# osmocom/osmo-trx

Hardware: AMD Instinct MI355X
Metric: Mbursts/s detect+demod (156.25 sym, 4 SPS) (higher is better)
Workload: dtype f32

## Files before the change

osmo_trx_amd/csrc/trx_device.h:

```cpp
#pragma once
#include <hip/hip_runtime.h>
#include <stdint.h>
#include <stdlib.h>
#include <atomic>

#include "trx_tables.h"
#include "../../include/trxhip.h"

#define WAVE 64
#define TRX_PAD 20
#define TRX_DEC_LEN 208
#define TRX_CORR_MAX 128
#define TRX_DEC_NARROW 160
#define TRX_CORR_NARROW 80
#define TRX_CZ_PAD 12
#define TRX_CZ_LEN (TRX_CZ_PAD + TRX_CORR_MAX + TRX_CZ_PAD)
#define TRX_SINCV_LDS (TRX_SINCV_LEN + 32)
#define TRX_CLIP_THRESH 30000.0f
#define TRX_WPB 12

#define LSEQ_TSC(s)   ((s) * 16)
#define LSEQ_RACH(i)  (128 + (i) * 40)
#define LSEQ_EDGE(s)  (248 + (s) * 16)
#define LSEQ_DUMMY    376
// ... 395 lines not shown
		p.y += v.y * w[u];
	}
	return p;
}

__device__ __forceinline__ int sinc_base_lo(int f) { return trx_sincv_swz(f); }
__device__ __forceinline__ int sinc_base_hi(int f) { return (f == 0) ? 512 : trx_sincv_swz(512 - f); }

__device__ __forceinline__ c32 interp_point(const c32 *cz, int ix512, const float *sincv)
{
	const int fl = ix512 >> 9;
	const int f = ix512 & 511;
	return interp_taps(cz + (fl - 7), sincv + sinc_base_lo(f), sincv + sinc_base_hi(f));
}

struct PeakConst {
	int flA;
	int loA, hiA;
	int offB;
	int ratio_off;
};
__device__ __forceinline__ int node_offset(int n, int inc0);
__device__ __forceinline__ PeakConst peak_const(int lane)
{
	PeakConst pc;
	const int offA = node_offset(lane >> 1, 256) + ((lane & 1) ? 1024 : 0);
	pc.flA = offA >> 9;
	pc.loA = sinc_base_lo(offA & 511);
	pc.hiA = sinc_base_hi(offA & 511);
	pc.offB = (lane < 32) ? node_offset(lane >> 1, 8) + ((lane & 1) ? 1024 : 0) : (2 * (lane & 15) - 15) + 512;
// ... 31 lines not shown
	int off = 0;
#pragma unroll
	for (int Lw = 0; Lw < LEVELS; Lw++) {
		const unsigned bit = 2u * node;
		const unsigned l = (unsigned)(lt >> bit) & 1u;
		stop |= (unsigned)(eq >> bit) & 1u;
		const int step = inc0 >> Lw;
		const int delta = l ? step : -step;
		off += stop ? 0 : delta;
		node = 2u * node + 1u + l;
	}
	tie = stop != 0u;
	return off;
}

__device__ __forceinline__ void peak_detect_spec(const c32 *cz, int max_idx, const float *sincv, const PeakConst &pc,
						  int lane, int *toa512_out, c32 *val_out, const float4 *wa4 = nullptr)
{
	int E = (max_idx - 1) * 512;
	bool tie = false;

	{
		const c32 *const ca = cz + ((max_idx - 1) + pc.flA - 7);
		const float nv = wa4 ? norm2(interp_taps_w(ca, wa4[lane], wa4[64 + lane], wa4[128 + lane], wa4[192 + lane]))
				     : norm2(interp_taps(ca, sincv + pc.loA, sincv + pc.hiA));
		E += walk_tree<5>(nv, 256, tie);
	}
	int final_ix;
	c32 val;
	if (!tie) {
		const c32 pv = interp_point(cz, E + pc.offB, sincv);
		const float nv = norm2(pv);
		const int offB = walk_tree<4>(nv, 8, tie);
		E += offB;
		final_ix = E + 512;
		const int src = 32 + ((offB + 15) >> 1);
		val.x = lane_val(pv.x, src);
		val.y = lane_val(pv.y, src);
	}
	if (tie) {
		final_ix = E + 512;
		val = interp_point(cz, final_ix, sincv);
	}
	*toa512_out = final_ix;
	*val_out = val;
}

#define TRX_FAST_W      2.6f
#define TRX_FAST_KAPPA  6e-6f
static __device__ unsigned long long g_trx_fast_stats[4];

__device__ __forceinline__ trx_v2f pk_fma_w(trx_v2f x, float w, trx_v2f acc)
{
	return __builtin_elementwise_fma(x, (trx_v2f){ w, w }, acc);
}

__device__ __forceinline__ c32 interp_taps_fma(const c32 *c, const float *sa, const float *sb)
// ... 506 lines not shown
```

osmo_trx_amd/csrc/trx_kernel_nb.hip:

```cpp
#include "trx_k4_common.h"
#include "trx_nb_asm.inc"

#define NB_D_LEN    160
#define NB_CZ_LEN   (TRX_CZ_PAD + TRX_CORR_NARROW + TRX_CZ_PAD)
#define NB_SLICE    (K4_XS + NB_D_LEN + NB_CZ_LEN)
#define NB_COMP_ROWS (TRX_DELAY_FILTS + 1)
#define NB_TABLES_FLOATS (TRX_SINCV_LDS + 16 * WAVE + NB_COMP_ROWS * 36 + 16 + 8 * 8 + 5 * WAVE + 5 * WAVE + 2 * 8 * 16)
#define NB_TABLES_BYTES (NB_TABLES_FLOATS * 4)
#define NB_WPB 16
#define NB_POOL_RING 64
#define NB_POOL_UNSET (-1)
#define NB_POOL_END (-2)
#define NB_NO_BURST 0xffffffffu
#define NB_LDS_TAIL (16 + 4 * NB_POOL_RING)
#define NB_LDS_BYTES (NB_TABLES_BYTES + NB_WPB * NB_SLICE * 8 + NB_LDS_TAIL)
#define NB_MAX_TOA 32



typedef float v3f __attribute__((ext_vector_type(3)));
typedef int v4i __attribute__((ext_vector_type(4)));
typedef __attribute__((address_space(3))) v2f lds_v2f;

template <typename T>
__device__ __forceinline__ unsigned lds_addr(const T *p)
{
	return (unsigned)(uintptr_t)(const __attribute__((address_space(3))) T *)p;
}

__device__ __forceinline__ int nb_lane_id()
{
	int lane;
	asm volatile("v_mbcnt_lo_u32_b32 %0, -1, 0\n\tv_mbcnt_hi_u32_b32 %0, -1, %0" : "=v"(lane));
	return lane;
}

// ... 19 lines not shown
	float *const wa4f = sincv + TRX_SINCV_LDS;
	const float4 *const wa4 = reinterpret_cast<const float4 *>(wa4f);
	float *const comp = wa4f + 16 * WAVE;
	float *const gdec = comp + NB_COMP_ROWS * 36;
	float *const lhdr = gdec + 16;
	int *const pkcl = reinterpret_cast<int *>(lhdr + 8 * 8);
	int *const lcn = pkcl + 5 * WAVE;
	c32 *const lseq = reinterpret_cast<c32 *>(lcn + 5 * WAVE);
	c32 *const wbase = reinterpret_cast<c32 *>(smem + NB_TABLES_BYTES) + (size_t)wave * NB_SLICE;
	int *const wg_next = reinterpret_cast<int *>(reinterpret_cast<c32 *>(smem + NB_TABLES_BYTES) + (size_t)NB_WPB * NB_SLICE);
	int *const pool_g = wg_next + 4;
	c32 *const P = wbase;
	c32 *const D = wbase + K4_XS;
	c32 *const cz = D + NB_D_LEN + TRX_CZ_PAD;

	for (int i = threadIdx.x; i < TRX_SINCV_LDS; i += blockDim.x)
		sincv[i] = (i < TRX_SINCV_LEN) ? tab->sincv[i] : 0.0f;
	for (int i = threadIdx.x; i < 16 * WAVE; i += blockDim.x) {
		const int l = i & (WAVE - 1), u = i >> 6;
		const PeakConst pcl = peak_const(l);
		const int q = (u < 8) ? pcl.loA + 512 * (7 - u) : pcl.hiA + 512 * (u - 8);
		wa4f[((u >> 2) * WAVE + l) * 4 + (u & 3)] = (q < TRX_SINCV_LEN) ? tab->sincv[q] : 0.0f;
	}
	for (int i = threadIdx.x; i < NB_COMP_ROWS * 36; i += blockDim.x) {
		const int f = i / 36, j = i % 36;
		comp[i] = (j >= TRX_FUSED_SH) ? tab->comp_filt[f][j - TRX_FUSED_SH] : 0.0f;
	}
	if (threadIdx.x < 16)
		gdec[threadIdx.x] = tab->dec_taps[threadIdx.x];
	if (threadIdx.x < 128)
		lseq[threadIdx.x] = make_float2(tab->seq[TRX_SEQ_TSC0 + (threadIdx.x >> 4)].taps[threadIdx.x & 15].re,
						tab->seq[TRX_SEQ_TSC0 + (threadIdx.x >> 4)].taps[threadIdx.x & 15].im);
	if (threadIdx.x < 64)
		lhdr[threadIdx.x] = reinterpret_cast<const float *>(&tab->seq[TRX_SEQ_TSC0 + (threadIdx.x >> 3)].gain)[threadIdx.x & 7];
	if (threadIdx.x < WAVE) {
		const PeakConst pc0 = peak_const(threadIdx.x);
		pkcl[0 * WAVE + threadIdx.x] = pc0.flA;
		pkcl[1 * WAVE + threadIdx.x] = pc0.loA;
		pkcl[2 * WAVE + threadIdx.x] = pc0.hiA;
		pkcl[3 * WAVE + threadIdx.x] = pc0.offB;
		pkcl[4 * WAVE + threadIdx.x] = pc0.ratio_off;
		lcn[0 * WAVE + threadIdx.x] = pc0.ratio_off * 8;
		lcn[1 * WAVE + threadIdx.x] = (pc0.flA - 8) * 8;
		lcn[2 * WAVE + threadIdx.x] = pc0.offB;
		const int l = threadIdx.x, e = (l - 52) / 3, t = (l - 52) % 3;
		const bool sp = l >= 52;
		lcn[3 * WAVE + l] = 8 * (sp ? (t == 0 ? e : t == 1 ? e + 3 : e - 3) : 4 + 3 * (l < 49 ? l : 49));
		lcn[4 * WAVE + l] = sp ? (e + (t == 2 ? 4 : 0)) * K4_NTP * 4 : -1;
	}
	for (int i = lane0; i < NB_SLICE; i += WAVE)
		wbase[i] = make_float2(0.0f, 0.0f);
	if (threadIdx.x == 0) {
		wg_next[0] = NB_WPB;
		wg_next[1] = 0;
	}
	if (threadIdx.x < NB_POOL_RING)
		pool_g[threadIdx.x] = NB_POOL_UNSET;
	__syncthreads();

	const float thr2 = thresh * thresh;
	float gkv = lane0 == 5 ? gk5 : lane0 == 6 ? gk6 : lane0 == 7 ? gk7 : gk8;
	asm volatile("" : "+v"(gkv));
// ... 338 lines not shown
			{
				int clip;
				asm("s_cmp_lg_u64 %1, 0\n\ts_cselect_b32 %0, 1, 0" : "=s"(clip) : "s"(__ballot(amax > TRX_CLIP_THRESH)) : "scc");

				const int len = 16 + (int)max_toa;
				__builtin_assume(len >= 16 && len <= 16 + NB_MAX_TOA);
				float v;
				const int lag0 = (len <= NB_ASM_CORR_MAX_LEN) ? NB_ASM_CORR_LANE0 : 0;
				asm volatile(NB_ASM_DECCORR
					     : [nrm] "=&v"(v)
					     : [aw] "v"(a_w), [zero] "v"(0), [len] "s"(len), [tsc] "s"(tsc)
					     : NB_ASM_CLOBBERS);
				{
					DIAG_MARK(3);
					int m_bits, es_bits, bidx;
					int kr, ka, kb, kic, ktp;
					asm volatile(NB_ASM_AMAX("ds_read_b32 %[kr], %[l4] offset:%c[lc]", "ds_read_b32 %[ka], %[l4] offset:%c[lc]+256",
								 "ds_read_b32 %[kb], %[l4] offset:%c[lc]+512", "ds_read_b32 %[kic], %[l4] offset:%c[lc]+768",
								 "ds_read_b32 %[ktp], %[l4] offset:%c[lc]+1024", "s_nop 0", "s_nop 0", "s_nop 0")
						     "s_sub_u32 %[bidx], %[bidx], %[lag0]\n\t"
						     "s_waitcnt lgkmcnt(0)"
						     : [m] "=&s"(m_bits), [es] "=&s"(es_bits), [bidx] "=&s"(bidx), [kr] "=&v"(kr), [ka] "=&v"(ka), [kb] "=&v"(kb),
						       [kic] "=&v"(kic), [ktp] "=&v"(ktp)
						     : [nrm] "v"(v), [ep] "v"(epart), [l4] "v"(a_l4), [lag0] "s"(lag0),
						       [lc] "n"((TRX_SINCV_LDS + 16 * WAVE + NB_COMP_ROWS * 36 + 16 + 64 + 5 * WAVE) * 4)
						     : NB_ASM_CLOBBERS);
					DIAG_MARK(4);
					int st, e512;
					float km;
					asm volatile(NB_ASM_DETA
						     : [st] "=&" NB_ASM_ST(st), [e] "=&s"(e512), [km] "=&v"(km)
						     : [bidx] "s"(bidx), [len] "s"(len), [czb] "s"(lds_addr(cz)), [kr] "v"(kr), [ka] "v"(ka), [l16] "v"(a_l16),
						       [gkv] "v"(gkv), [c0] "v"(gc0)
						     : NB_ASM_CLOBBERS_ST);
					DIAG_MARK(5);
					int toa512 = 0, xr_bits = 0, xi_bits = 0;
					if (__builtin_expect(st == 1, 1)) {
						asm volatile(NB_ASM_DETB
							     : [st] "=&" NB_ASM_ST(st), [toa] "=&s"(toa512), [xr] "=&s"(xr_bits), [xi] "=&s"(xi_bits)
							     : [e] "s"(e512), [kb] "v"(kb), [czb] "s"(lds_addr(cz)), [km] "v"(km)
							     : NB_ASM_CLOBBERS_ST);
						DIAG_MARK(6);
					}
					if (__builtin_expect(st != 1, 0)) {
						int stc = st;
						asm volatile("" : "+s"(stc));
						if (stc == 3) {
							const int lane = nb_lane_id();
							if (lane == 0)
								atomicAdd(&g_trx_fast_stats[0], 1ull);
							PeakConst pkc;
							pkc.flA = pkcl[0 * WAVE + lane]; pkc.loA = pkcl[1 * WAVE + lane]; pkc.hiA = pkcl[2 * WAVE + lane];
							pkc.offB = pkcl[3 * WAVE + lane]; pkc.ratio_off = pkcl[4 * WAVE + lane];
							c32 xcorr;
							peak_detect_spec(cz, bidx, sincv, pkc, lane, &toa512, &xcorr, wa4);
							toa512 = uni(toa512);
							xr_bits = uni(__float_as_int(xcorr.x));
							xi_bits = uni(__float_as_int(xcorr.y));
							st = 1;
						} else if (stc == 2) {
							if (nb_lane_id() == 0) atomicAdd(&g_trx_fast_stats[2], 1ull);
							mark_left(b);
							keep = 0;
						} else {
							const float energy = __int_as_float(es_bits) * 0.0125f;
							const float rssi = rssi_db(full_scale, energy);
							const uint32_t flags = ((uint32_t)clip << 8) | (1u << 16);
							int word = clip ? -TRXHIP_SIGERR_CLIP : 0;
							word = put_lane<1>(word, 0.0f);
							word = put_lane<2>(word, 0.0f);
// ... 5 lines not shown
							recw = word;
							o = (v3f){ 0.0f, 0.0f, 0.0f };
							pend_rm = 0xff;
						}
					}
					if (__builtin_expect(st == 1, 1)) {
						int ok, s_bits;
						float d0, d1, d2;
						const int t5 = (t5pk << (28 - 4 * tsc)) >> 28;
						asm volatile("s_setprio 0");
						asm volatile(NB_ASM_TAIL
							     : [ok] "=&s"(ok), [ssum] "=&s"(s_bits), [d0] "=&v"(d0), [d1] "=&v"(d1), [d2] "=&v"(d2)
							     : [toa] "s"(toa512), [xr] "s"(xr_bits), [xi] "s"(xi_bits), [t5] "s"(t5), [hdrb] "s"(lds_addr(lhdr) + 32u * (unsigned)tsc),
							       [e8lo] "s"((unsigned)e8_addr), [e8hi] "s"((unsigned)(e8_addr >> 32)), [l16] "v"(a_l16),
							       [aw] "v"(a_w), [pb] "s"(lds_addr(P)), [cb] "s"(lds_addr(comp) + 4u * (K4_U0 + TRX_FUSED_SH)), [db] "s"(lds_addr(D)),
							       [kic] "v"(kic), [ktp] "v"(ktp)
							     : NB_ASM_CLOBBERS);
						DIAG_MARK(10);
						asm volatile("s_setprio 2");
						o.x = __builtin_amdgcn_fmed3f(fmaf(0.5f, d0, 0.5f), 0.0f, 1.0f);
						o.y = __builtin_amdgcn_fmed3f(fmaf(0.5f, d1, 0.5f), 0.0f, 1.0f);
						o.z = __builtin_amdgcn_fmed3f(fmaf(0.5f, d2, 0.5f), 0.0f, 1.0f);
						queue_record(xr_bits, xi_bits, es_bits, toa512 - t5 - 10 * 512, s_bits,
							     (int)((uint32_t)tsc | ((uint32_t)clip << 8) | (37u << 24)), b);
						if (__builtin_expect(!ok, 0)) {
							const int lane = nb_lane_id();
							if (lane == 0) atomicAdd(&g_trx_fast_stats[3], 1ull);
							const float *const h = lhdr + 8 * tsc;
							const float xr = __int_as_float(xr_bits), xi = __int_as_float(xi_bits);
							const float a0 = xr * h[2], a1 = xr * h[3], a2 = xi * h[3], a3 = xi * h[2];
							const c32 ampv = make_float2(unif(a0 - a2), unif(a1 + a3));
							if (!demod_general(t5 + 10 * 512 - toa512, ampv, lane)) {
								q_n--;
								mark_left(b);
								keep = 0;
							}
						}
// ... 28 lines not shown
```

osmo_trx_amd/csrc/trx_nb_asm.inc:

```
#define NB_ASM_GDEC_OFF 29968
#define NB_ASM_LSEQ_OFF 32848
#define NB_ASM_DEC_MAX_NACT 60
#define NB_ASM_CORR_LANE0 19
#define NB_ASM_CORR_MAX_LEN 45
#define NB_ASM_AW_PD 512
#define NB_ASM_AW_D 5760
#define NB_ASM_AW_CZ 7136
#define NB_ASM_ST "{s98}"
#define NB_ASM_CLOBBERS "v64", "v65", "v66", "v67", "v68", "v69", "v70", "v71", "v72", "v73", "v74", "v75", "v76", "v77", "v78", "v79", "v80", "v81", "v82", "v83", "v84", "v85", "v86", "v87", "v88", "v89", "v90", "v91", "v92", "v93", "v94", "v95", "v96", "v97", "v98", "v99", "v100", "v101", "v102", "v103", "v104", "v105", "v106", "v107", "v108", "v109", "v110", "v111", "v112", "v113", "v114", "v115", "v116", "v117", "v118", "v119", "v120", "v121", "v122", "v123", "v124", "v125", "v126", "v127", "s87", "s88", "s89", "s90", "s91", "s92", "s93", "s94", "s95", "s96", "s97", "s98", "s99", "vcc", "scc", "memory"
#define NB_ASM_CLOBBERS_ST "v64", "v65", "v66", "v67", "v68", "v69", "v70", "v71", "v72", "v73", "v74", "v75", "v76", "v77", "v78", "v79", "v80", "v81", "v82", "v83", "v84", "v85", "v86", "v87", "v88", "v89", "v90", "v91", "v92", "v93", "v94", "v95", "v96", "v97", "v98", "v99", "v100", "v101", "v102", "v103", "v104", "v105", "v106", "v107", "v108", "v109", "v110", "v111", "v112", "v113", "v114", "v115", "v116", "v117", "v118", "v119", "v120", "v121", "v122", "v123", "v124", "v125", "v126", "v127", "s87", "s88", "s89", "s90", "s91", "s92", "s93", "s94", "s95", "s96", "s97", "s99", "vcc", "scc", "memory"
#define NB_ASM_DECCORR \
	"s_add_u32 s92, %[len], 15\n\t" \
	"s_cmp_gt_u32 %[len], 45\n\t" \
	"s_cbranch_scc1 .Lnbc_dc_wide\n\t" \
	"s_sub_u32 s88, 60, s92\n\t" \
	"s_lshr_b64 exec, -1, s88\n\t" \
	"ds_read_b128 v[120:123], %[zero] offset:29968\n\t" \
	"ds_read_b128 v[124:127], %[zero] offset:29984\n\t" \
	"ds_read_b64 v[98:99], %[aw] offset:1952\n\t" \
	"ds_read_b64 v[100:101], %[aw] offset:3392\n\t" \
	"ds_read_b64 v[102:103], %[aw] offset:4832\n\t" \
	"ds_read_b64 v[96:97], %[aw] offset:512\n\t" \
	"s_waitcnt lgkmcnt(3)\n\t" \
	"v_pk_mul_f32 v[64:65], v[98:99], v[120:121] op_sel:[0,0] op_sel_hi:[1,0]\n\t" \
// ... 1278 lines not shown
	".Lnb_da_end:\n\t"
#define NB_ASM_DETB \
	"v_mov_b64_e32 v[64:65], 0\n\t" \
	"v_mov_b64_e32 v[66:67], 0\n\t" \
	"v_add_u32_e32 v68, %[e], %[kb]\n\t" \
	"s_add_u32 s88, %[czb], -56\n\t" \
	"s_mov_b32 exec_lo, 0x3fffffff\n\t" \
	"s_mov_b32 exec_hi, 0xffff\n\t" \
	"v_ashrrev_i32_e32 v69, 9, v68\n\t" \
	"v_and_b32_e32 v70, 0x1ff, v68\n\t" \
	"v_lshl_add_u32 v69, v69, 3, s88\n\t" \
	"v_bfe_u32 v71, v70, 4, 5\n\t" \
	"v_sub_u32_e32 v72, 0x200, v70\n\t" \
	"v_xor_b32_e32 v71, v71, v70\n\t" \
	"v_bfe_u32 v73, v72, 4, 5\n\t" \
	"v_lshlrev_b32_e32 v71, 2, v71\n\t" \
	"v_xor_b32_e32 v72, v73, v72\n\t" \
	"v_lshlrev_b32_e32 v72, 2, v72\n\t" \
	"ds_read_b64 v[80:81], v69 offset:0\n\t" \
	"ds_read_b32 v96, v71 offset:14336\n\t" \
	"ds_read_b64 v[82:83], v69 offset:8\n\t" \
	"ds_read_b32 v97, v71 offset:12288\n\t" \
	"ds_read_b64 v[84:85], v69 offset:16\n\t" \
	"ds_read_b32 v98, v71 offset:10240\n\t" \
	"ds_read_b64 v[86:87], v69 offset:24\n\t" \
	"ds_read_b32 v99, v71 offset:8192\n\t" \
	"ds_read_b64 v[88:89], v69 offset:32\n\t" \
	"ds_read_b32 v100, v71 offset:6144\n\t" \
	"ds_read_b64 v[90:91], v69 offset:40\n\t" \
	"ds_read_b32 v101, v71 offset:4096\n\t" \
	"ds_read_b64 v[92:93], v69 offset:48\n\t" \
	"ds_read_b32 v102, v71 offset:2048\n\t" \
	"ds_read_b64 v[94:95], v69 offset:56\n\t" \
	"ds_read_b32 v103, v71 offset:0\n\t" \
	"s_waitcnt lgkmcnt(12)\n\t" \
	"v_pk_fma_f32 v[64:65], v[80:81], v[96:97], v[64:65] op_sel:[0,0,0] op_sel_hi:[1,0,1]\n\t" \
	"v_pk_fma_f32 v[66:67], v[82:83], v[96:97], v[66:67] op_sel:[0,1,0] op_sel_hi:[1,1,1]\n\t" \
	"ds_read_b64 v[104:105], v69 offset:64\n\t" \
	"ds_read_b32 v120, v72 offset:0\n\t" \
	"ds_read_b64 v[106:107], v69 offset:72\n\t" \
	"ds_read_b32 v121, v72 offset:2048\n\t" \
	"s_waitcnt lgkmcnt(12)\n\t" \
	"v_pk_fma_f32 v[64:65], v[84:85], v[98:99], v[64:65] op_sel:[0,0,0] op_sel_hi:[1,0,1]\n\t" \
	"v_pk_fma_f32 v[66:67], v[86:87], v[98:99], v[66:67] op_sel:[0,1,0] op_sel_hi:[1,1,1]\n\t" \
	"ds_read_b64 v[108:109], v69 offset:80\n\t" \
	"ds_read_b32 v122, v72 offset:4096\n\t" \
	"ds_read_b64 v[110:111], v69 offset:88\n\t" \
	"ds_read_b32 v123, v72 offset:6144\n\t" \
	"s_waitcnt lgkmcnt(12)\n\t" \
	"v_pk_fma_f32 v[64:65], v[88:89], v[100:101], v[64:65] op_sel:[0,0,0] op_sel_hi:[1,0,1]\n\t" \
	"v_pk_fma_f32 v[66:67], v[90:91], v[100:101], v[66:67] op_sel:[0,1,0] op_sel_hi:[1,1,1]\n\t" \
	"ds_read_b64 v[112:113], v69 offset:96\n\t" \
	"ds_read_b32 v124, v72 offset:8192\n\t" \
	"ds_read_b64 v[114:115], v69 offset:104\n\t" \
	"ds_read_b32 v125, v72 offset:10240\n\t" \
	"s_waitcnt lgkmcnt(12)\n\t" \
	"v_pk_fma_f32 v[64:65], v[92:93], v[102:103], v[64:65] op_sel:[0,0,0] op_sel_hi:[1,0,1]\n\t" \
	"v_pk_fma_f32 v[66:67], v[94:95], v[102:103], v[66:67] op_sel:[0,1,0] op_sel_hi:[1,1,1]\n\t" \
	"ds_read_b64 v[116:117], v69 offset:112\n\t" \
	"ds_read_b32 v126, v72 offset:12288\n\t" \
	"ds_read_b64 v[118:119], v69 offset:120\n\t" \
	"ds_read_b32 v127, v72 offset:14336\n\t" \
	"s_waitcnt lgkmcnt(12)\n\t" \
	"v_pk_fma_f32 v[64:65], v[104:105], v[120:121], v[64:65] op_sel:[0,0,0] op_sel_hi:[1,0,1]\n\t" \
	"v_pk_fma_f32 v[66:67], v[106:107], v[120:121], v[66:67] op_sel:[0,1,0] op_sel_hi:[1,1,1]\n\t" \
	"s_waitcnt lgkmcnt(8)\n\t" \
	"v_pk_fma_f32 v[64:65], v[108:109], v[122:123], v[64:65] op_sel:[0,0,0] op_sel_hi:[1,0,1]\n\t" \
	"v_pk_fma_f32 v[66:67], v[110:111], v[122:123], v[66:67] op_sel:[0,1,0] op_sel_hi:[1,1,1]\n\t" \
	"s_waitcnt lgkmcnt(4)\n\t" \
	"v_pk_fma_f32 v[64:65], v[112:113], v[124:125], v[64:65] op_sel:[0,0,0] op_sel_hi:[1,0,1]\n\t" \
	"v_pk_fma_f32 v[66:67], v[114:115], v[124:125], v[66:67] op_sel:[0,1,0] op_sel_hi:[1,1,1]\n\t" \
	"s_waitcnt lgkmcnt(0)\n\t" \
	"v_pk_fma_f32 v[64:65], v[116:117], v[126:127], v[64:65] op_sel:[0,0,0] op_sel_hi:[1,0,1]\n\t" \
	"v_pk_fma_f32 v[66:67], v[118:119], v[126:127], v[66:67] op_sel:[0,1,0] op_sel_hi:[1,1,1]\n\t" \
	"s_mov_b64 exec, -1\n\t" \
	"v_pk_add_f32 v[74:75], v[64:65], v[66:67]\n\t" \
	"s_add_u32 s92, %[e], 497\n\t" \
	"v_pk_mul_f32 v[76:77], v[74:75], v[74:75]\n\t" \
	"s_mov_b32 s98, 1\n\t" \
	"v_add_f32_e32 v78, v77, v76\n\t" \
	"v_fmamk_f32 v79, v78, 0x36c9539c, %[km]\n\t" \
	"v_sub_f32_e32 v96, v78, v79\n\t" \
	"v_add_f32_e32 v97, v78, v79\n\t" \
	"s_nop 0\n\t" \
// ... 18 lines not shown
	"s_bitcmp1_b32 s88, s95\n\t" \
	"s_addc_u32 s94, s94, s94\n\t" \
	".Lnb_db_walked:\n\t" \
	"s_add_u32 s93, s94, 32\n\t" \
	"s_lshl1_add_u32 %[toa], s94, s92\n\t" \
	"v_readlane_b32 %[xr], v74, s93\n\t" \
	"v_readlane_b32 %[xi], v75, s93\n\t" \
	".Lnb_db_end:\n\t"
#define NB_ASM_TAIL \
	"v_mov_b32_e32 v65, %[hdrb]\n\t" \
	"ds_read_b128 v[68:71], v65\n\t" \
	"s_sub_u32 s88, %[t5], %[toa]\n\t" \
	"s_add_u32 s87, s88, 5120\n\t" \
	"s_mov_b32 %[ok], 0\n\t" \
	"s_and_b32 s91, s87, 127\n\t" \
	"s_lshr_b32 s92, s91, 1\n\t" \
	"s_cmp_ge_u32 s91, 2\n\t" \
	"s_cselect_b32 s92, s92, 64\n\t" \
	"s_mul_i32 s93, s92, 768\n\t" \
	"s_add_u32 s94, %[e8lo], s93\n\t" \
	"s_addc_u32 s95, %[e8hi], 0\n\t" \
	"s_abs_i32 s96, %[toa]\n\t" \
	"s_add_u32 s96, s96, 256\n\t" \
	"global_load_dwordx4 v[120:123], %[l16], s[94:95]\n\t" \
	"s_lshr_b32 s96, s96, 9\n\t" \
	"s_sub_u32 s97, 0, s96\n\t" \
	"s_cmp_lt_i32 %[toa], 0\n\t" \
	"s_cselect_b32 s96, s97, s96\n\t" \
	"s_lshl_b32 s96, s96, 3\n\t" \
	"v_add_u32_e32 v64, s96, %[aw]\n\t" \
	"s_bfm_b64 exec, 16, 0\n\t" \
	"ds_read_b64 v[66:67], v64 offset:5760\n\t" \
	"s_mov_b64 exec, -1\n\t" \
	"s_waitcnt lgkmcnt(1)\n\t" \
// ... 8 lines not shown
	"v_add_f32_e32 v89, v89, v90\n\t" \
	"v_rcp_f32_e32 v89, v89\n\t" \
	"s_mov_b32 s88, 0xaaaaaaaa\n\t" \
	"s_mov_b32 s89, 0xaaaaaaaa\n\t" \
	"v_mul_f32_e32 v91, v86, v89\n\t" \
	"v_mul_f32_e64 v92, -v87, v89\n\t" \
	"v_cndmask_b32_e64 v119, v91, v92, s[88:89]\n\t" \
	"s_mov_b32 s88, 0xcccccccc\n\t" \
	"s_mov_b32 s89, 0xcccccccc\n\t" \
	"v_cndmask_b32_e64 v119, v119, -v119, s[88:89]\n\t" \
	"s_bfm_b64 exec, 16, 0\n\t" \
	"s_waitcnt lgkmcnt(0)\n\t" \
	"v_pk_mul_f32 v[66:67], v[66:67], v[66:67]\n\t" \
	"s_ashr_i32 s88, s87, 7\n\t" \
	"v_add_f32_e32 v81, v67, v66\n\t" \
	"s_and_b32 s89, s87, 127\n\t" \
	"s_lshr_b32 s90, s89, 1\n\t" \
	"v_add_f32_dpp v81, v81, v81 quad_perm:[1,0,3,2] row_mask:0xf bank_mask:0xf\n\t" \
	"s_cmp_ge_u32 s89, 2\n\t" \
	"s_cselect_b32 s90, s90, 64\n\t" \
	"v_add_f32_dpp v81, v81, v81 quad_perm:[2,3,0,1] row_mask:0xf bank_mask:0xf\n\t" \
	"s_sub_u32 s91, -18, s88\n\t" \
	"s_and_b32 s92, s91, 3\n\t" \
	"v_add_f32_dpp v81, v81, v81 row_half_mirror row_mask:0xf bank_mask:0xf\n\t" \
	"s_ashr_i32 s93, s91, 2\n\t" \
	"s_mul_i32 s94, s92, 180\n\t" \
	"v_add_f32_dpp v81, v81, v81 row_mirror row_mask:0xf bank_mask:0xf\n\t" \
	"s_add_u32 s94, s94, s93\n\t" \
	"s_lshl3_add_u32 s94, s94, %[pb]\n\t" \
	"v_mul_f32_e32 v81, 0x3d800000, v81\n\t" \
	"s_mul_i32 s95, s90, 144\n\t" \
	"s_add_u32 s95, s95, %[cb]\n\t" \
	"v_readlane_b32 %[ssum], v81, 0\n\t" \
	"s_mov_b64 exec, -1\n\t" \
	"s_sub_u32 s96, 0, s88\n\t" \
	"s_cmp_gt_u32 s96, 36\n\t" \
	"s_cbranch_scc1 .Lnbc_tl_wait\n\t" \
	"s_mov_b32 %[ok], 1\n\t" \
	"v_add_u32_e32 v112, s94, %[kic]\n\t" \
	"s_add_u32 s96, s92, 1\n\t" \
	"s_lshr_b32 s96, s96, 2\n\t" \
	"s_mul_i32 s96, s96, -5752\n\t" \
	"s_add_u32 s96, s96, 1440\n\t" \
	"v_add_u32_e32 v113, s96, v112\n\t" \
	"s_add_u32 s96, s92, 2\n\t" \
	"s_lshr_b32 s96, s96, 2\n\t" \
	"s_mul_i32 s96, s96, -5752\n\t" \
	"s_add_u32 s96, s96, 2880\n\t" \
	"v_add_u32_e32 v114, s96, v112\n\t" \
	"s_add_u32 s96, s92, 3\n\t" \
	"s_lshr_b32 s96, s96, 2\n\t" \
	"s_mul_i32 s96, s96, -5752\n\t" \
	"s_add_u32 s96, s96, 4320\n\t" \
	"v_add_u32_e32 v115, s96, v112\n\t" \
	"ds_read_b64 v[72:73], v112 offset:96\n\t" \
	"ds_read_b64 v[74:75], v113 offset:96\n\t" \
	"ds_read_b64 v[76:77], v114 offset:96\n\t" \
	"ds_read_b64 v[78:79], v115 offset:96\n\t" \
	"ds_read_b64 v[80:81], v112 offset:104\n\t" \
	"ds_read_b64 v[82:83], v113 offset:104\n\t" \
	"ds_read_b64 v[84:85], v114 offset:104\n\t" \
	"ds_read_b64 v[86:87], v115 offset:104\n\t" \
	"ds_read_b64 v[88:89], v112 offset:112\n\t" \
	"ds_read_b64 v[90:91], v113 offset:112\n\t" \
	"ds_read_b64 v[92:93], v114 offset:112\n\t" \
	"ds_read_b64 v[94:95], v115 offset:112\n\t" \
	"v_add_u32_e32 v116, %[db], %[l16]\n\t" \
	"v_cmp_lt_i32_e32 vcc, -1, %[ktp]\n\t" \
	"v_add_u32_e32 v117, %[db], %[ktp]\n\t" \
	"v_mov_b32_e32 v118, s95\n\t" \
	"v_mov_b64_e32 v[64:65], 0\n\t" \
	"v_mov_b64_e32 v[66:67], 0\n\t" \
	"v_mov_b64_e32 v[68:69], 0\n\t" \
	"v_cndmask_b32_e32 v117, v118, v117, vcc\n\t" \
	"s_waitcnt vmcnt(0)\n\t" \
	"ds_write_b128 v116, v[120:123]\n\t" \
	"ds_read_b128 v[96:99], v117 offset:0\n\t" \
	"ds_read_b128 v[100:103], v117 offset:16\n\t" \
	"ds_read_b128 v[104:107], v117 offset:32\n\t" \
	"ds_read_b128 v[108:111], v117 offset:48\n\t" \
	"ds_read_b128 v[124:127], v117 offset:64\n\t" \
// ... 90 lines not shown
	"v_pk_fma_f32 v[68:69], v[84:85], v[122:123], v[68:69] op_sel:[0,0,0] op_sel_hi:[1,0,1]\n\t" \
	"v_mov_b32_dpp v64, v64 wave_shr:1 row_mask:0xf bank_mask:0xf bound_ctrl:0\n\t" \
	"v_mov_b32_dpp v65, v65 wave_shr:1 row_mask:0xf bank_mask:0xf bound_ctrl:0\n\t" \
	"v_pk_fma_f32 v[66:67], v[78:79], v[122:123], v[66:67] op_sel:[0,1,0] op_sel_hi:[1,1,1]\n\t" \
	"v_pk_fma_f32 v[68:69], v[86:87], v[122:123], v[68:69] op_sel:[0,1,0] op_sel_hi:[1,1,1]\n\t" \
	"s_mov_b32 exec_lo, 0\n\t" \
	"s_mov_b32 exec_hi, 0xfff00000\n\t" \
	"v_pk_add_f32 v[64:65], v[64:65], v[66:67]\n\t" \
	"s_mov_b64 exec, -1\n\t" \
	"v_mul_f32_dpp %[d1], v119, v66 quad_perm:[3,2,1,0] row_mask:0xf bank_mask:0xf\n\t" \
	"v_mul_f32_dpp %[d2], v119, v68 quad_perm:[0,3,2,1] row_mask:0xf bank_mask:0xf\n\t" \
	"v_mul_f32_dpp %[d0], v119, v64 quad_perm:[2,1,0,3] row_mask:0xf bank_mask:0xf\n\t" \
	"v_fmac_f32_dpp %[d1], v119, v67 quad_perm:[2,1,0,3] row_mask:0xf bank_mask:0xf\n\t" \
	"v_fmac_f32_dpp %[d2], v119, v69 quad_perm:[3,2,1,0] row_mask:0xf bank_mask:0xf\n\t" \
	"v_fmac_f32_dpp %[d0], v119, v65 quad_perm:[1,0,3,2] row_mask:0xf bank_mask:0xf\n\t" \
	".Lnb_tl_end:\n\t"
#define NB_ASM_FIRG \
	"s_ashr_i32 s88, %[nk], 7\n\t" \
	"s_and_b32 s89, %[nk], 127\n\t" \
	"s_lshr_b32 s90, s89, 1\n\t" \
	"s_cmp_ge_u32 s89, 2\n\t" \
	"s_cselect_b32 s90, s90, 64\n\t" \
	"s_sub_u32 s91, -18, s88\n\t" \
	"s_and_b32 s92, s91, 3\n\t" \
	"s_ashr_i32 s93, s91, 2\n\t" \
	"s_mul_i32 s94, s92, 180\n\t" \
	"s_add_u32 s94, s94, s93\n\t" \
	"s_lshl3_add_u32 s94, s94, %[pb]\n\t" \
	"s_mul_i32 s95, s90, 144\n\t" \
	"s_add_u32 s95, s95, %[cb]\n\t" \
// ... 235 lines not shown
```

osmo_trx_amd/csrc/trx_tables.h:

```cpp
#pragma once
#include <stddef.h>
#include <stdint.h>

struct trx_c32 { float re, im; };

#define TRX_FUSED_U0 6
#define TRX_FUSED_NT 24
#define TRX_FUSED_SH ((4 - TRX_FUSED_U0 % 4) % 4)
#define TRX_FUSED_NTP ((TRX_FUSED_NT + 3) / 4 * 4)

enum {
	TRX_SEQ_TSC0   = 0,
	TRX_SEQ_RACH0  = 8,
	TRX_SEQ_DUMMY  = 11,
	TRX_SEQ_EDGE0  = 12,
	TRX_SEQ_SCH    = 20,
	TRX_NSEQ       = 21,
	TRX_SEQ_MAXLEN = 64,
	TRX_SINCV_LEN  = 4096,
	TRX_DELAY_FILTS = 64,
	TRX_DELAY_HLEN = 20,
};

struct trx_seq {
// ... 37 lines not shown

#define TRX_IFLAG_NO_UNIT 0x40
#define TRX_IFLAG_NO_SYM  0x80
#define TRX_IFLAG_NO_FAST 0x20
#define TRX_REDO_HDR 16

#define TRX_TABLES_MAGIC   0x54585254u
#define TRX_TABLES_VERSION 8u

static inline
#ifdef __HIPCC__
__host__ __device__
#endif
int trx_sincv_swz(int q) { return q ^ ((q >> 4) & 31); }

int trx_tables_generate(trx_tables *out);

void trx_polyphase_taps(unsigned p, unsigned q, unsigned filt_len, float bw, float *out);
```

Baseline: 1172.

## Interleave sinc LUT row pairs in LDS for 64-bit loads and fold clamps into asm

Rearranges the sinc interpolation table in LDS so adjacent tap rows are interleaved in pairs. Each ds_read_b64 now fetches two tap weights, halving the weight loads in the peak-interpolation asm and the C++ fallback path. It also packs the lane constant table so two values come from one 64-bit read, simplifies the filter-row address arithmetic with compare-select, and moves the output clamp into the asm as fused clamped FMAs. The change touches many hand-tuned waitcnt counts and offsets, so any mismatch could silently corrupt results.

```diff
diff --git a/osmo_trx_amd/csrc/trx_device.h b/osmo_trx_amd/csrc/trx_device.h
--- a/osmo_trx_amd/csrc/trx_device.h
+++ b/osmo_trx_amd/csrc/trx_device.h
@@ -433,6 +433,38 @@
 	return interp_taps(cz + (fl - 7), sincv + sinc_base_lo(f), sincv + sinc_base_hi(f));
 }
 
+__device__ __forceinline__ c32 interp_taps_pairs(const c32 *c, const float *sincp, int sa, int sb)
+{
+	typedef const volatile trx_v2f __attribute__((address_space(3))) *lds_ptr;
+	lds_ptr cp = (lds_ptr)c;
+	asm("" : "+v"(cp));
+	c32 p = make_float2(0.0f, 0.0f);
+#pragma unroll
+	for (int u = 0; u < 8; u++) {
+		const trx_v2f v = cp[u];
+		const float w = sincp[trx_sincp_idx(7 - u, sa)];
+		p.x += v.x * w;
+		p.y += v.y * w;
+	}
+#pragma unroll
+	for (int u = 0; u < 8; u++) {
+		const trx_v2f v = cp[8 + u];
+		const float w = sincp[trx_sincp_idx(u, sb)];
+		p.x += v.x * w;
+		p.y += v.y * w;
+	}
+	return p;
+}
+
+template <bool PAIRS>
+__device__ __forceinline__ c32 interp_point_l(const c32 *cz, int ix512, const float *sincv)
+{
+	if (!PAIRS)
+		return interp_point(cz, ix512, sincv);
+	const int fl = ix512 >> 9, f = ix512 & 511;
+	return interp_taps_pairs(cz + (fl - 7), sincv, sinc_base_lo(f), sinc_base_hi(f));
+}
+
 struct PeakConst {
 	int flA;
 	int loA, hiA;
@@ -494,6 +526,7 @@
 	return off;
 }
 
+template <bool PAIRS = false>
 __device__ __forceinline__ void peak_detect_spec(const c32 *cz, int max_idx, const float *sincv, const PeakConst &pc,
 						  int lane, int *toa512_out, c32 *val_out, const float4 *wa4 = nullptr)
 {
@@ -503,13 +536,14 @@
 	{
 		const c32 *const ca = cz + ((max_idx - 1) + pc.flA - 7);
 		const float nv = wa4 ? norm2(interp_taps_w(ca, wa4[lane], wa4[64 + lane], wa4[128 + lane], wa4[192 + lane]))
-				     : norm2(interp_taps(ca, sincv + pc.loA, sincv + pc.hiA));
+				     : PAIRS ? norm2(interp_taps_pairs(ca, sincv, pc.loA, pc.hiA))
+					     : norm2(interp_taps(ca, sincv + pc.loA, sincv + pc.hiA));
 		E += walk_tree<5>(nv, 256, tie);
 	}
 	int final_ix;
 	c32 val;
 	if (!tie) {
-		const c32 pv = interp_point(cz, E + pc.offB, sincv);
+		const c32 pv = interp_point_l<PAIRS>(cz, E + pc.offB, sincv);
 		const float nv = norm2(pv);
 		const int offB = walk_tree<4>(nv, 8, tie);
 		E += offB;
@@ -520,7 +554,7 @@
 	}
 	if (tie) {
 		final_ix = E + 512;
-		val = interp_point(cz, final_ix, sincv);
+		val = interp_point_l<PAIRS>(cz, final_ix, sincv);
 	}
 	*toa512_out = final_ix;
 	*val_out = val;
diff --git a/osmo_trx_amd/csrc/trx_kernel_nb.hip b/osmo_trx_amd/csrc/trx_kernel_nb.hip
--- a/osmo_trx_amd/csrc/trx_kernel_nb.hip
+++ b/osmo_trx_amd/csrc/trx_kernel_nb.hip
@@ -20,6 +20,7 @@
 
 typedef float v3f __attribute__((ext_vector_type(3)));
 typedef int v4i __attribute__((ext_vector_type(4)));
+typedef int v2i __attribute__((ext_vector_type(2)));
 typedef __attribute__((address_space(3))) v2f lds_v2f;
 
 template <typename T>
@@ -69,8 +70,11 @@
 	c32 *const D = wbase + K4_XS;
 	c32 *const cz = D + NB_D_LEN + TRX_CZ_PAD;
 
-	for (int i = threadIdx.x; i < TRX_SINCV_LDS; i += blockDim.x)
-		sincv[i] = (i < TRX_SINCV_LEN) ? tab->sincv[i] : 0.0f;
+	static_assert(4 * TRX_SINCP_STRIDE <= TRX_SINCV_LDS, "the row pairs fit the LUT's LDS space");
+	for (int i = threadIdx.x; i < TRX_SINCV_LDS; i += blockDim.x) {
+		const int src = trx_sincp_src(i);
+		sincv[i] = (src >= 0) ? tab->sincv[src] : 0.0f;
+	}
 	for (int i = threadIdx.x; i < 16 * WAVE; i += blockDim.x) {
 		const int l = i & (WAVE - 1), u = i >> 6;
 		const PeakConst pcl = peak_const(l);
@@ -95,12 +99,12 @@
 		pkcl[2 * WAVE + threadIdx.x] = pc0.hiA;
 		pkcl[3 * WAVE + threadIdx.x] = pc0.offB;
 		pkcl[4 * WAVE + threadIdx.x] = pc0.ratio_off;
-		lcn[0 * WAVE + threadIdx.x] = pc0.ratio_off * 8;
-		lcn[1 * WAVE + threadIdx.x] = (pc0.flA - 8) * 8;
-		lcn[2 * WAVE + threadIdx.x] = pc0.offB;
+		lcn[2 * threadIdx.x + 0] = pc0.ratio_off * 8;
+		lcn[2 * threadIdx.x + 1] = (pc0.flA - 8) * 8;
+		lcn[2 * (WAVE + threadIdx.x) + 0] = pc0.offB;
 		const int l = threadIdx.x, e = (l - 52) / 3, t = (l - 52) % 3;
 		const bool sp = l >= 52;
-		lcn[3 * WAVE + l] = 8 * (sp ? (t == 0 ? e : t == 1 ? e + 3 : e - 3) : 4 + 3 * (l < 49 ? l : 49));
+		lcn[2 * (WAVE + l) + 1] = 8 * (sp ? (t == 0 ? e : t == 1 ? e + 3 : e - 3) : 4 + 3 * (l < 49 ? l : 49));
 		lcn[4 * WAVE + l] = sp ? (e + (t == 2 ? 4 : 0)) * K4_NTP * 4 : -1;
 	}
 	for (int i = lane0; i < NB_SLICE; i += WAVE)
@@ -469,14 +473,14 @@
 				{
 					DIAG_MARK(3);
 					int m_bits, es_bits, bidx;
-					int kr, ka, kb, kic, ktp;
-					asm volatile(NB_ASM_AMAX("ds_read_b32 %[kr], %[l4] offset:%c[lc]", "ds_read_b32 %[ka], %[l4] offset:%c[lc]+256",
-								 "ds_read_b32 %[kb], %[l4] offset:%c[lc]+512", "ds_read_b32 %[kic], %[l4] offset:%c[lc]+768",
-								 "ds_read_b32 %[ktp], %[l4] offset:%c[lc]+1024", "s_nop 0", "s_nop 0", "s_nop 0")
+					v2i kra, kbc;
+					int ktp;
+					asm volatile(NB_ASM_AMAX("v_lshlrev_b32_e32 v90, 1, %[l4]", "ds_read_b64 %[kra], v90 offset:%c[lc]",
+								 "ds_read_b64 %[kbc], v90 offset:%c[lc]+512", "ds_read_b32 %[ktp], %[l4] offset:%c[lc]+1024",
+								 "s_nop 0", "s_nop 0", "s_nop 0", "s_nop 0")
 						     "s_sub_u32 %[bidx], %[bidx], %[lag0]\n\t"
 						     "s_waitcnt lgkmcnt(0)"
-						     : [m] "=&s"(m_bits), [es] "=&s"(es_bits), [bidx] "=&s"(bidx), [kr] "=&v"(kr), [ka] "=&v"(ka), [kb] "=&v"(kb),
-						       [kic] "=&v"(kic), [ktp] "=&v"(ktp)
+						     : [m] "=&s"(m_bits), [es] "=&s"(es_bits), [bidx] "=&s"(bidx), [kra] "=&v"(kra), [kbc] "=&v"(kbc), [ktp] "=&v"(ktp)
 						     : [nrm] "v"(v), [ep] "v"(epart), [l4] "v"(a_l4), [lag0] "s"(lag0),
 						       [lc] "n"((TRX_SINCV_LDS + 16 * WAVE + NB_COMP_ROWS * 36 + 16 + 64 + 5 * WAVE) * 4)
 						     : NB_ASM_CLOBBERS);
@@ -485,7 +489,7 @@
 					float km;
 					asm volatile(NB_ASM_DETA
 						     : [st] "=&" NB_ASM_ST(st), [e] "=&s"(e512), [km] "=&v"(km)
-						     : [bidx] "s"(bidx), [len] "s"(len), [czb] "s"(lds_addr(cz)), [kr] "v"(kr), [ka] "v"(ka), [l16] "v"(a_l16),
+						     : [bidx] "s"(bidx), [len] "s"(len), [czb] "s"(lds_addr(cz)), [kr] "v"(kra.x), [ka] "v"(kra.y), [l16] "v"(a_l16),
 						       [gkv] "v"(gkv), [c0] "v"(gc0)
 						     : NB_ASM_CLOBBERS_ST);
 					DIAG_MARK(5);
@@ -493,7 +497,7 @@
 					if (__builtin_expect(st == 1, 1)) {
 						asm volatile(NB_ASM_DETB
 							     : [st] "=&" NB_ASM_ST(st), [toa] "=&s"(toa512), [xr] "=&s"(xr_bits), [xi] "=&s"(xi_bits)
-							     : [e] "s"(e512), [kb] "v"(kb), [czb] "s"(lds_addr(cz)), [km] "v"(km)
+							     : [e] "s"(e512), [kb] "v"(kbc.x), [czb] "s"(lds_addr(cz)), [km] "v"(km)
 							     : NB_ASM_CLOBBERS_ST);
 						DIAG_MARK(6);
 					}
@@ -508,7 +512,7 @@
 							pkc.flA = pkcl[0 * WAVE + lane]; pkc.loA = pkcl[1 * WAVE + lane]; pkc.hiA = pkcl[2 * WAVE + lane];
 							pkc.offB = pkcl[3 * WAVE + lane]; pkc.ratio_off = pkcl[4 * WAVE + lane];
 							c32 xcorr;
-							peak_detect_spec(cz, bidx, sincv, pkc, lane, &toa512, &xcorr, wa4);
+							peak_detect_spec<true>(cz, bidx, sincv, pkc, lane, &toa512, &xcorr, wa4);
 							toa512 = uni(toa512);
 							xr_bits = uni(__float_as_int(xcorr.x));
 							xi_bits = uni(__float_as_int(xcorr.y));
@@ -544,13 +548,13 @@
 							     : [toa] "s"(toa512), [xr] "s"(xr_bits), [xi] "s"(xi_bits), [t5] "s"(t5), [hdrb] "s"(lds_addr(lhdr) + 32u * (unsigned)tsc),
 							       [e8lo] "s"((unsigned)e8_addr), [e8hi] "s"((unsigned)(e8_addr >> 32)), [l16] "v"(a_l16),
 							       [aw] "v"(a_w), [pb] "s"(lds_addr(P)), [cb] "s"(lds_addr(comp) + 4u * (K4_U0 + TRX_FUSED_SH)), [db] "s"(lds_addr(D)),
-							       [kic] "v"(kic), [ktp] "v"(ktp)
+							       [kic] "v"(kbc.y), [ktp] "v"(ktp)
 							     : NB_ASM_CLOBBERS);
 						DIAG_MARK(10);
 						asm volatile("s_setprio 2");
-						o.x = __builtin_amdgcn_fmed3f(fmaf(0.5f, d0, 0.5f), 0.0f, 1.0f);
-						o.y = __builtin_amdgcn_fmed3f(fmaf(0.5f, d1, 0.5f), 0.0f, 1.0f);
-						o.z = __builtin_amdgcn_fmed3f(fmaf(0.5f, d2, 0.5f), 0.0f, 1.0f);
+						o.x = d0;
+						o.y = d1;
+						o.z = d2;
 						queue_record(xr_bits, xi_bits, es_bits, toa512 - t5 - 10 * 512, s_bits,
 							     (int)((uint32_t)tsc | ((uint32_t)clip << 8) | (37u << 24)), b);
 						if (__builtin_expect(!ok, 0)) {
diff --git a/osmo_trx_amd/csrc/trx_nb_asm.inc b/osmo_trx_amd/csrc/trx_nb_asm.inc
--- a/osmo_trx_amd/csrc/trx_nb_asm.inc
+++ b/osmo_trx_amd/csrc/trx_nb_asm.inc
@@ -1316,60 +1316,52 @@
 	"v_sub_u32_e32 v72, 0x200, v70\n\t" \
 	"v_xor_b32_e32 v71, v71, v70\n\t" \
 	"v_bfe_u32 v73, v72, 4, 5\n\t" \
-	"v_lshlrev_b32_e32 v71, 2, v71\n\t" \
+	"v_lshlrev_b32_e32 v71, 3, v71\n\t" \
 	"v_xor_b32_e32 v72, v73, v72\n\t" \
-	"v_lshlrev_b32_e32 v72, 2, v72\n\t" \
+	"v_lshlrev_b32_e32 v72, 3, v72\n\t" \
 	"ds_read_b64 v[80:81], v69 offset:0\n\t" \
-	"ds_read_b32 v96, v71 offset:14336\n\t" \
+	"ds_read_b64 v[96:97], v71 offset:12312\n\t" \
 	"ds_read_b64 v[82:83], v69 offset:8\n\t" \
-	"ds_read_b32 v97, v71 offset:12288\n\t" \
 	"ds_read_b64 v[84:85], v69 offset:16\n\t" \
-	"ds_read_b32 v98, v71 offset:10240\n\t" \
+	"ds_read_b64 v[98:99], v71 offset:8208\n\t" \
 	"ds_read_b64 v[86:87], v69 offset:24\n\t" \
-	"ds_read_b32 v99, v71 offset:8192\n\t" \
 	"ds_read_b64 v[88:89], v69 offset:32\n\t" \
-	"ds_read_b32 v100, v71 offset:6144\n\t" \
+	"ds_read_b64 v[100:101], v71 offset:4104\n\t" \
 	"ds_read_b64 v[90:91], v69 offset:40\n\t" \
-	"ds_read_b32 v101, v71 offset:4096\n\t" \
 	"ds_read_b64 v[92:93], v69 offset:48\n\t" \
-	"ds_read_b32 v102, v71 offset:2048\n\t" \
+	"ds_read_b64 v[102:103], v71 offset:0\n\t" \
 	"ds_read_b64 v[94:95], v69 offset:56\n\t" \
-	"ds_read_b32 v103, v71 offset:0\n\t" \
-	"s_waitcnt lgkmcnt(12)\n\t" \
-	"v_pk_fma_f32 v[64:65], v[80:81], v[96:97], v[64:65] op_sel:[0,0,0] op_sel_hi:[1,0,1]\n\t" \
-	"v_pk_fma_f32 v[66:67], v[82:83], v[96:97], v[66:67] op_sel:[0,1,0] op_sel_hi:[1,1,1]\n\t" \
+	"s_waitcnt lgkmcnt(9)\n\t" \
+	"v_pk_fma_f32 v[64:65], v[80:81], v[96:97], v[64:65] op_sel:[0,1,0] op_sel_hi:[1,1,1]\n\t" \
+	"v_pk_fma_f32 v[66:67], v[82:83], v[96:97], v[66:67] op_sel:[0,0,0] op_sel_hi:[1,0,1]\n\t" \
 	"ds_read_b64 v[104:105], v69 offset:64\n\t" \
-	"ds_read_b32 v120, v72 offset:0\n\t" \
+	"ds_read_b64 v[120:121], v72 offset:0\n\t" \
 	"ds_read_b64 v[106:107], v69 offset:72\n\t" \
-	"ds_read_b32 v121, v72 offset:2048\n\t" \
-	"s_waitcnt lgkmcnt(12)\n\t" \
-	"v_pk_fma_f32 v[64:65], v[84:85], v[98:99], v[64:65] op_sel:[0,0,0] op_sel_hi:[1,0,1]\n\t" \
-	"v_pk_fma_f32 v[66:67], v[86:87], v[98:99], v[66:67] op_sel:[0,1,0] op_sel_hi:[1,1,1]\n\t" \
+	"s_waitcnt lgkmcnt(9)\n\t" \
+	"v_pk_fma_f32 v[64:65], v[84:85], v[98:99], v[64:65] op_sel:[0,1,0] op_sel_hi:[1,1,1]\n\t" \
+	"v_pk_fma_f32 v[66:67], v[86:87], v[98:99], v[66:67] op_sel:[0,0,0] op_sel_hi:[1,0,1]\n\t" \
 	"ds_read_b64 v[108:109], v69 offset:80\n\t" \
-	"ds_read_b32 v122, v72 offset:4096\n\t" \
+	"ds_read_b64 v[122:123], v72 offset:4104\n\t" \
 	"ds_read_b64 v[110:111], v69 offset:88\n\t" \
-	"ds_read_b32 v123, v72 offset:6144\n\t" \
-	"s_waitcnt lgkmcnt(12)\n\t" \
-	"v_pk_fma_f32 v[64:65], v[88:89], v[100:101], v[64:65] op_sel:[0,0,0] op_sel_hi:[1,0,1]\n\t" \
-	"v_pk_fma_f32 v[66:67], v[90:91], v[100:101], v[66:67] op_sel:[0,1,0] op_sel_hi:[1,1,1]\n\t" \
+	"s_waitcnt lgkmcnt(9)\n\t" \
+	"v_pk_fma_f32 v[64:65], v[88:89], v[100:101], v[64:65] op_sel:[0,1,0] op_sel_hi:[1,1,1]\n\t" \
+	"v_pk_fma_f32 v[66:67], v[90:91], v[100:101], v[66:67] op_sel:[0,0,0] op_sel_hi:[1,0,1]\n\t" \
 	"ds_read_b64 v[112:113], v69 offset:96\n\t" \
-	"ds_read_b32 v124, v72 offset:8192\n\t" \
+	"ds_read_b64 v[124:125], v72 offset:8208\n\t" \
 	"ds_read_b64 v[114:115], v69 offset:104\n\t" \
-	"ds_read_b32 v125, v72 offset:10240\n\t" \
-	"s_waitcnt lgkmcnt(12)\n\t" \
-	"v_pk_fma_f32 v[64:65], v[92:93], v[102:103], v[64:65] op_sel:[0,0,0] op_sel_hi:[1,0,1]\n\t" \
-	"v_pk_fma_f32 v[66:67], v[94:95], v[102:103], v[66:67] op_sel:[0,1,0] op_sel_hi:[1,1,1]\n\t" \
+	"s_waitcnt lgkmcnt(9)\n\t" \
+	"v_pk_fma_f32 v[64:65], v[92:93], v[102:103], v[64:65] op_sel:[0,1,0] op_sel_hi:[1,1,1]\n\t" \
+	"v_pk_fma_f32 v[66:67], v[94:95], v[102:103], v[66:67] op_sel:[0,0,0] op_sel_hi:[1,0,1]\n\t" \
 	"ds_read_b64 v[116:117], v69 offset:112\n\t" \
-	"ds_read_b32 v126, v72 offset:12288\n\t" \
+	"ds_read_b64 v[126:127], v72 offset:12312\n\t" \
 	"ds_read_b64 v[118:119], v69 offset:120\n\t" \
-	"ds_read_b32 v127, v72 offset:14336\n\t" \
-	"s_waitcnt lgkmcnt(12)\n\t" \
+	"s_waitcnt lgkmcnt(9)\n\t" \
 	"v_pk_fma_f32 v[64:65], v[104:105], v[120:121], v[64:65] op_sel:[0,0,0] op_sel_hi:[1,0,1]\n\t" \
 	"v_pk_fma_f32 v[66:67], v[106:107], v[120:121], v[66:67] op_sel:[0,1,0] op_sel_hi:[1,1,1]\n\t" \
-	"s_waitcnt lgkmcnt(8)\n\t" \
+	"s_waitcnt lgkmcnt(6)\n\t" \
 	"v_pk_fma_f32 v[64:65], v[108:109], v[122:123], v[64:65] op_sel:[0,0,0] op_sel_hi:[1,0,1]\n\t" \
 	"v_pk_fma_f32 v[66:67], v[110:111], v[122:123], v[66:67] op_sel:[0,1,0] op_sel_hi:[1,1,1]\n\t" \
-	"s_waitcnt lgkmcnt(4)\n\t" \
+	"s_waitcnt lgkmcnt(3)\n\t" \
 	"v_pk_fma_f32 v[64:65], v[112:113], v[124:125], v[64:65] op_sel:[0,0,0] op_sel_hi:[1,0,1]\n\t" \
 	"v_pk_fma_f32 v[66:67], v[114:115], v[124:125], v[66:67] op_sel:[0,1,0] op_sel_hi:[1,1,1]\n\t" \
 	"s_waitcnt lgkmcnt(0)\n\t" \
@@ -1418,10 +1410,10 @@
 	"s_add_u32 s87, s88, 5120\n\t" \
 	"s_mov_b32 %[ok], 0\n\t" \
 	"s_and_b32 s91, s87, 127\n\t" \
-	"s_lshr_b32 s92, s91, 1\n\t" \
+	"s_lshr_b32 s99, s91, 1\n\t" \
 	"s_cmp_ge_u32 s91, 2\n\t" \
-	"s_cselect_b32 s92, s92, 64\n\t" \
-	"s_mul_i32 s93, s92, 768\n\t" \
+	"s_cselect_b32 s99, s99, 64\n\t" \
+	"s_mul_i32 s93, s99, 768\n\t" \
 	"s_add_u32 s94, %[e8lo], s93\n\t" \
 	"s_addc_u32 s95, %[e8hi], 0\n\t" \
 	"s_abs_i32 s96, %[toa]\n\t" \
@@ -1460,57 +1452,47 @@
 	"v_pk_mul_f32 v[66:67], v[66:67], v[66:67]\n\t" \
 	"s_ashr_i32 s88, s87, 7\n\t" \
 	"v_add_f32_e32 v81, v67, v66\n\t" \
-	"s_and_b32 s89, s87, 127\n\t" \
-	"s_lshr_b32 s90, s89, 1\n\t" \
-	"v_add_f32_dpp v81, v81, v81 quad_perm:[1,0,3,2] row_mask:0xf bank_mask:0xf\n\t" \
-	"s_cmp_ge_u32 s89, 2\n\t" \
-	"s_cselect_b32 s90, s90, 64\n\t" \
-	"v_add_f32_dpp v81, v81, v81 quad_perm:[2,3,0,1] row_mask:0xf bank_mask:0xf\n\t" \
 	"s_sub_u32 s91, -18, s88\n\t" \
 	"s_and_b32 s92, s91, 3\n\t" \
-	"v_add_f32_dpp v81, v81, v81 row_half_mirror row_mask:0xf bank_mask:0xf\n\t" \
+	"v_add_f32_dpp v81, v81, v81 quad_perm:[1,0,3,2] row_mask:0xf bank_mask:0xf\n\t" \
 	"s_ashr_i32 s93, s91, 2\n\t" \
 	"s_mul_i32 s94, s92, 180\n\t" \
-	"v_add_f32_dpp v81, v81, v81 row_mirror row_mask:0xf bank_mask:0xf\n\t" \
+	"v_add_f32_dpp v81, v81, v81 quad_perm:[2,3,0,1] row_mask:0xf bank_mask:0xf\n\t" \
 	"s_add_u32 s94, s94, s93\n\t" \
 	"s_lshl3_add_u32 s94, s94, %[pb]\n\t" \
+	"v_add_f32_dpp v81, v81, v81 row_half_mirror row_mask:0xf bank_mask:0xf\n\t" \
+	"s_mul_i32 s95, s99, 144\n\t" \
+	"s_add_u32 s95, s95, %[cb]\n\t" \
+	"v_add_f32_dpp v81, v81, v81 row_mirror row_mask:0xf bank_mask:0xf\n\t" \
 	"v_mul_f32_e32 v81, 0x3d800000, v81\n\t" \
-	"s_mul_i32 s95, s90, 144\n\t" \
-	"s_add_u32 s95, s95, %[cb]\n\t" \
+	"s_sub_u32 s96, 0, s88\n\t" \
 	"v_readlane_b32 %[ssum], v81, 0\n\t" \
 	"s_mov_b64 exec, -1\n\t" \
-	"s_sub_u32 s96, 0, s88\n\t" \
 	"s_cmp_gt_u32 s96, 36\n\t" \
 	"s_cbranch_scc1 .Lnbc_tl_wait\n\t" \
 	"s_mov_b32 %[ok], 1\n\t" \
 	"v_add_u32_e32 v112, s94, %[kic]\n\t" \
-	"s_add_u32 s96, s92, 1\n\t" \
-	"s_lshr_b32 s96, s96, 2\n\t" \
-	"s_mul_i32 s96, s96, -5752\n\t" \
-	"s_add_u32 s96, s96, 1440\n\t" \
+	"s_cmp_gt_u32 s92, 2\n\t" \
+	"s_cselect_b32 s96, -5752, 0\n\t" \
 	"v_add_u32_e32 v113, s96, v112\n\t" \
-	"s_add_u32 s96, s92, 2\n\t" \
-	"s_lshr_b32 s96, s96, 2\n\t" \
-	"s_mul_i32 s96, s96, -5752\n\t" \
-	"s_add_u32 s96, s96, 2880\n\t" \
+	"s_cmp_gt_u32 s92, 1\n\t" \
+	"s_cselect_b32 s96, -5752, 0\n\t" \
 	"v_add_u32_e32 v114, s96, v112\n\t" \
-	"s_add_u32 s96, s92, 3\n\t" \
-	"s_lshr_b32 s96, s96, 2\n\t" \
-	"s_mul_i32 s96, s96, -5752\n\t" \
-	"s_add_u32 s96, s96, 4320\n\t" \
+	"s_cmp_gt_u32 s92, 0\n\t" \
+	"s_cselect_b32 s96, -5752, 0\n\t" \
 	"v_add_u32_e32 v115, s96, v112\n\t" \
 	"ds_read_b64 v[72:73], v112 offset:96\n\t" \
-	"ds_read_b64 v[74:75], v113 offset:96\n\t" \
-	"ds_read_b64 v[76:77], v114 offset:96\n\t" \
-	"ds_read_b64 v[78:79], v115 offset:96\n\t" \
+	"ds_read_b64 v[74:75], v113 offset:1536\n\t" \
+	"ds_read_b64 v[76:77], v114 offset:2976\n\t" \
+	"ds_read_b64 v[78:79], v115 offset:4416\n\t" \
 	"ds_read_b64 v[80:81], v112 offset:104\n\t" \
-	"ds_read_b64 v[82:83], v113 offset:104\n\t" \
-	"ds_read_b64 v[84:85], v114 offset:104\n\t" \
-	"ds_read_b64 v[86:87], v115 offset:104\n\t" \
+	"ds_read_b64 v[82:83], v113 offset:1544\n\t" \
+	"ds_read_b64 v[84:85], v114 offset:2984\n\t" \
+	"ds_read_b64 v[86:87], v115 offset:4424\n\t" \
 	"ds_read_b64 v[88:89], v112 offset:112\n\t" \
-	"ds_read_b64 v[90:91], v113 offset:112\n\t" \
-	"ds_read_b64 v[92:93], v114 offset:112\n\t" \
-	"ds_read_b64 v[94:95], v115 offset:112\n\t" \
+	"ds_read_b64 v[90:91], v113 offset:1552\n\t" \
+	"ds_read_b64 v[92:93], v114 offset:2992\n\t" \
+	"ds_read_b64 v[94:95], v115 offset:4432\n\t" \
 	"v_add_u32_e32 v116, %[db], %[l16]\n\t" \
 	"v_cmp_lt_i32_e32 vcc, -1, %[ktp]\n\t" \
 	"v_add_u32_e32 v117, %[db], %[ktp]\n\t" \
@@ -1631,6 +1613,9 @@
 	"v_fmac_f32_dpp %[d1], v119, v67 quad_perm:[2,1,0,3] row_mask:0xf bank_mask:0xf\n\t" \
 	"v_fmac_f32_dpp %[d2], v119, v69 quad_perm:[3,2,1,0] row_mask:0xf bank_mask:0xf\n\t" \
 	"v_fmac_f32_dpp %[d0], v119, v65 quad_perm:[1,0,3,2] row_mask:0xf bank_mask:0xf\n\t" \
+	"v_fma_f32 %[d1], %[d1], 0.5, 0.5 clamp\n\t" \
+	"v_fma_f32 %[d2], %[d2], 0.5, 0.5 clamp\n\t" \
+	"v_fma_f32 %[d0], %[d0], 0.5, 0.5 clamp\n\t" \
 	".Lnb_tl_end:\n\t"
 #define NB_ASM_FIRG \
 	"s_ashr_i32 s88, %[nk], 7\n\t" \
diff --git a/osmo_trx_amd/csrc/trx_tables.h b/osmo_trx_amd/csrc/trx_tables.h
--- a/osmo_trx_amd/csrc/trx_tables.h
+++ b/osmo_trx_amd/csrc/trx_tables.h
@@ -75,6 +75,27 @@
 #endif
 int trx_sincv_swz(int q) { return q ^ ((q >> 4) & 31); }
 
+#define TRX_SINCP_STRIDE 1026
+static inline
+#ifdef __HIPCC__
+__host__ __device__
+#endif
+int trx_sincp_idx(int row, int slot) { return (row >> 1) * TRX_SINCP_STRIDE + 2 * slot + (row & 1); }
+static inline
+#ifdef __HIPCC__
+__host__ __device__
+#endif
+int trx_sincp_src(int i)
+{
+	const int pair = i / TRX_SINCP_STRIDE, rem = i % TRX_SINCP_STRIDE;
+	const int row = 2 * pair + (rem & 1), slot = rem >> 1;
+	if (pair >= 4)
+		return -1;
+	if (slot < 512)
+		return 512 * row + slot;
+	return (row + 1 < 8) ? 512 * (row + 1) : -1;
+}
+
 int trx_tables_generate(trx_tables *out);
 
 void trx_polyphase_taps(unsigned p, unsigned q, unsigned filt_len, float bw, float *out);
```

New measurement: 1185, median of 6. 1.01x the previous value.
